# USharma002/CUDA-PathTracer

Hardware: AMD Instinct MI355X
Metric: Msamples/s (higher is better)
Workload: dtype f32; 1 GPU; c2: cbox.obj 1024x1024, 256 spp, max_depth 8, default camera, seed 2023 (BASELINE configs[1]); width=1024, height=1024, spp=256, max_depth=8, segments_per_launch=default, parallelism=tile1, frames=one ptmi_render_frame call per step

## Files before the change

cuda-pathtracer_amd/csrc/bounce.h:

```cpp
#pragma once
#include "shading.h"
#include "sweep_records.h"

namespace ptmi {

struct BounceArgs {
    DeviceScene sc; TileMap tm; PathState st; FrameParams fp;
    const int* queue_in; int n_in;
    const int* count_in;
    int* queue_out; int* count_out;
    int segments;
    StatCounters* stats;
    int many_waves;
    int* done_count;
    int* next_count;
    int* host_count;
    int* cursor;
    unsigned int* cost; unsigned int* cost_max;
};

using BounceKernel = void (*)(BounceArgs);
#pragma GCC visibility push(hidden)
BounceKernel select_bounce_sync(const BounceArgs& a);
BounceKernel select_bounce_phased(const BounceArgs& a);
BounceKernel select_bounce_wide(const BounceArgs& a);
#pragma GCC visibility pop

inline bool is_guided(const BounceArgs& a) { return a.fp.sampling_mode != 0 && a.sc.cdfs != nullptr; }

#ifdef PTMI_TRACE_WAVES
#define PTMI_TR(...) __VA_ARGS__
#else
#define PTMI_TR(...)
#endif

template <bool LDS_GEOM, bool SWEEP_RECORDS = false>
__device__ __forceinline__ float4* stage_scene(const DeviceScene& sc, float4* lds, const float4*& nodes, const float4*& prims, const float4*& mats) {
    static_assert(LDS_GEOM || !SWEEP_RECORDS, "the sweep's records exist in LDS only");
    nodes = sc.nodes; prims = sc.prims; mats = sc.mats;
    if (LDS_GEOM) {
        const int n_node_vec = 2 * sc.n_nodes, n_prim_vec = sc.prim_stride * sc.n_prims, n_mat_vec = 3 * sc.n_prims;
        if (SWEEP_RECORDS) {
            ptmi_sweep_prepare(reinterpret_cast<const ptmi_vec_bits*>(sc.nodes), sc.n_nodes, reinterpret_cast<const ptmi_vec_bits*>(sc.prims),
                               sc.prim_stride, sc.n_prims, reinterpret_cast<ptmi_vec_bits*>(lds), reinterpret_cast<ptmi_vec_bits*>(lds + n_node_vec),
                               lds_address(lds), (int)threadIdx.x, kBlock);
        } else {
            for (int i = threadIdx.x; i < n_node_vec; i += kBlock) lds[i] = sc.nodes[i];
            for (int i = threadIdx.x; i < n_prim_vec; i += kBlock) lds[n_node_vec + i] = sc.prims[i];
        }
        for (int i = threadIdx.x; i < n_mat_vec; i += kBlock) lds[n_node_vec + n_prim_vec + i] = sc.mats[i];
        nodes = lds; prims = lds + n_node_vec; mats = lds + n_node_vec + n_prim_vec;
        lds += n_node_vec + n_prim_vec + n_mat_vec;
        __syncthreads();
    }
    return lds;
}

template <bool STATS, bool COMPACT = true>
__device__ __forceinline__ void finish_launch(const BounceArgs& a, bool alive, int slot, const LaneCounters& cn) {
    if (COMPACT) {
        const unsigned long long mask = __ballot(alive);
        const int lane = threadIdx.x & 63;
        int base = 0;
        if (lane == 0 && mask) base = atomicAdd(a.count_out, __popcll(mask));
        base = __shfl(base, 0);
        if (alive) a.queue_out[base + __popcll(mask & ((1ull << lane) - 1ull))] = slot;
    }
    if (STATS) {
        unsigned long long r = cn.rays, nv = cn.node_visits, pt = cn.prim_tests, h = cn.hits, tv = cn.top_visits;
        unsigned long long cc = cn.cert_chain, cf = cn.cert_fallback;
        for (int off = 32; off > 0; off >>= 1) {
            r += __shfl_down(r, off); nv += __shfl_down(nv, off); pt += __shfl_down(pt, off); h += __shfl_down(h, off); tv += __shfl_down(tv, off);
            cc += __shfl_down(cc, off); cf += __shfl_down(cf, off);
        }
        if ((threadIdx.x & 63) == 0) {
            atomicAdd(&a.stats->rays, r); atomicAdd(&a.stats->node_visits, nv);
            atomicAdd(&a.stats->prim_tests, pt); atomicAdd(&a.stats->hits, h);
            if (tv) atomicAdd(&a.stats->top_node_visits, tv);
            if (cc) atomicAdd(&a.stats->cert_chain, cc);
            if (cf) atomicAdd(&a.stats->cert_fallback, cf);
        }
    }
}

__device__ __forceinline__ void publish_count(const BounceArgs& a) {
    if (!a.host_count) return;
    if ((threadIdx.x & 63) == 0) {
        __threadfence();
        if (atomicAdd(a.done_count, 1) == (int)(gridDim.x * (kBlock / 64)) - 1) {
            const int c = atomicAdd(a.count_out, 0);
            atomicExch(a.next_count, 0); atomicExch(a.next_count + 1, 0);
            atomicExch(a.done_count, 0);
            __hip_atomic_store(a.host_count, c, __ATOMIC_RELEASE, __HIP_MEMORY_SCOPE_SYSTEM);
        }
    }
}

__device__ __forceinline__ bool end_visit(const BounceArgs& a, int n_in, bool more, int& slot, PathRegs& p, int& segs_left) {
    store_path(a.st, slot, p);
    if (a.cost) {
        const unsigned int c = a.cost[slot] + (unsigned int)(a.segments - segs_left);
        a.cost[slot] = c;
        if (!more) atomicMax(a.cost_max, c);
    }
    const int lane = threadIdx.x & 63;
    const unsigned long long ending = __ballot(1), surviving = __ballot(more);
    const int first = __ffsll((long long)ending) - 1;
    int out_base = 0, in_base = 0;
    if (lane == first) {
        if (surviving) out_base = atomicAdd(a.count_out, __popcll(surviving));
        if (a.cursor) in_base = atomicAdd(a.cursor, __popcll(ending));
    }
    out_base = __shfl(out_base, first); in_base = __shfl(in_base, first);
    if (more) a.queue_out[out_base + __popcll(surviving & ((1ull << lane) - 1ull))] = slot;
    const int entry = (int)(gridDim.x * kBlock) + in_base + __popcll(ending & ((1ull << lane) - 1ull));
    if (!(a.cursor && entry < n_in)) return false;
    slot = a.queue_in ? a.queue_in[entry] : entry;
    load_path(a.st, a.tm, slot, p);
    segs_left = a.segments;
    return true;
}

}
```

cuda-pathtracer_amd/csrc/bounce_sync.hip:

```cpp
#include "bounce.h"

namespace ptmi {

template <int MODE, bool LDS_GEOM, bool HAS_QUADS, bool STATS, bool GUIDED, bool BATCH>
__device__ __forceinline__ void bounce_body(const BounceArgs& a) {
    extern __shared__ float4 smem[];
    static_assert(MODE != TRAVERSAL_SWEEP || LDS_GEOM, "the sweep reads the scene through LDS broadcasts");
    const int n_in = a.count_in ? *a.count_in : a.n_in;
    if ((int)(blockIdx.x * kBlock) >= n_in) return;
    const int idx = blockIdx.x * kBlock + threadIdx.x;
    const bool active = idx < n_in;
    const float4 *nodes, *prims, *mats;
    float4* lds = stage_scene<LDS_GEOM, MODE == TRAVERSAL_SWEEP>(a.sc, smem, nodes, prims, mats);
    int* stack = reinterpret_cast<int*>(lds) + threadIdx.x;
    if (GUIDED) fill_grid_solid_angles();

    const int slot = active ? (a.queue_in ? a.queue_in[idx] : idx) : 0;
    bool alive = active;
    PathRegs p = {};
    if (active) load_path(a.st, a.tm, slot, p);
    LaneCounters cn = {0, 0, 0, 0, 0, 0, 0};

    for (int seg = 0; seg < a.segments; seg++) {
        if (!__any(alive)) break;
        float t = 0.0f; int k = -1;
        if (STATS && alive) cn.rays++;
        const bool hit = scene_intersect<MODE, HAS_QUADS, STATS>(nodes, prims, a.sc.prim_stride, a.sc.n_nodes, stack, alive,
                                                               p.o, p.d, 1e-4f, FLT_MAX, t, k, cn);
        constexpr bool LEAN = MODE == TRAVERSAL_SWEEP && !STATS && !GUIDED;
        if (alive) alive = shade_step<STATS, GUIDED, false, BATCH, LEAN>(a.fp, a.tm, MatSource{mats, nullptr, nullptr}, a.sc.cdfs, p, hit, t, k, cn, slot);
    }

    if (active) store_path(a.st, slot, p);
    finish_launch<STATS>(a, alive, slot, cn);
}
template <int MODE, bool LDS_GEOM, bool HAS_QUADS, bool STATS, bool GUIDED, bool BATCH>
__global__ __launch_bounds__(kBlock, GUIDED ? 6 : ((BATCH || (HAS_QUADS && !STATS)) && MODE == TRAVERSAL_SWEEP ? 8 : 1)) __attribute__((amdgpu_num_sgpr(80))) void ptmi_bounce(BounceArgs a) {
    bounce_body<MODE, LDS_GEOM, HAS_QUADS, STATS, GUIDED, BATCH>(a);
    publish_count(a);
}

BounceKernel select_bounce_sync(const BounceArgs& a) {
    const auto pick = [&](auto mode, auto geom) {
        return with_bool(a.sc.has_quads, [&](auto quads) {
            return with_bool(a.stats != nullptr, [&](auto stats) {
                return with_bool(is_guided(a), [&](auto guided) {
                    return with_bool(a.fp.n_frames > 1, [&](auto batch) -> BounceKernel {
                        return ptmi_bounce<decltype(mode)::value, decltype(geom)::value, decltype(quads)::value, decltype(stats)::value,
                                           decltype(guided)::value, decltype(batch)::value>;
                    });
                });
            });
        });
    };
    switch (a.sc.traversal) {
        case TRAVERSAL_SWEEP: return pick(std::integral_constant<int, TRAVERSAL_SWEEP>{}, std::true_type{});
        case TRAVERSAL_LANE: return with_bool(a.sc.lds_resident, [&](auto geom) { return pick(std::integral_constant<int, TRAVERSAL_LANE>{}, geom); });
        default: return with_bool(a.sc.lds_resident, [&](auto geom) { return pick(std::integral_constant<int, TRAVERSAL_STACK>{}, geom); });
    }
}

}
```

cuda-pathtracer_amd/csrc/kernels.hip:

```cpp
#include "bounce.h"

namespace ptmi {

__global__ __launch_bounds__(kBlock) void ptmi_render_init(TileMap tm, PathState st, const uint32_t* __restrict__ jump,
                                                           unsigned long long seed_base) {
    __shared__ uint32_t M[160 * 5];
    const int n = tm.local_rows * tm.width;
    const int slot = blockIdx.x * kBlock + threadIdx.x;
    const bool live = slot < n;
    int x = 0, y = 0;
    const unsigned int pix = live ? (unsigned int)global_pixel(tm, slot, x, y) : 0u;
    const unsigned long long seed = seed_base + (unsigned long long)pix;
    const uint32_t s0 = ((uint32_t)seed) ^ 0xaad26b49u;
    const uint32_t s1 = (uint32_t)(seed >> 32) ^ 0xf7dcefddu;
    const uint32_t t0 = 1099087573u * s0;
    const uint32_t t1 = 2591861531u * s1;
    uint32_t v[5] = {123456789u + t0, 362436069u ^ t0, 521288629u + t1, 88675123u ^ t1, 5783321u + t0};
    const uint32_t d = 6615241u + t1 + t0;

    for (int k = 0; k < 32; k++) {
        const bool mine = live && ((pix >> k) & 1u);
        if (!__syncthreads_or(mine ? 1 : 0)) continue;
        for (int i = threadIdx.x; i < 160 * 5; i += kBlock) M[i] = jump[k * 160 * 5 + i];
        __syncthreads();
        if (mine) {
            uint32_t r[5] = {0u, 0u, 0u, 0u, 0u};
#pragma unroll
            for (int w = 0; w < 5; w++) {
                const uint32_t word = v[w];
                for (int b = 0; b < 32; b++) {
                    const uint32_t m = 0u - ((word >> b) & 1u);
                    const uint32_t* row = &M[(w * 32 + b) * 5];
                    r[0] ^= row[0] & m; r[1] ^= row[1] & m; r[2] ^= row[2] & m; r[3] ^= row[3] & m; r[4] ^= row[4] & m;
                }
            }
#pragma unroll
            for (int w = 0; w < 5; w++) v[w] = r[w];
        }
        __syncthreads();
    }
    if (!live) return;
    st.E[slot] = make_uint4(v[0], v[1], v[2], v[3]);
    st.F[slot] = make_uint2(v[4], d);
    st.A[slot] = make_float4(0, 0, 0, 1.0f);
    st.B[slot] = make_float4(0, 0, 1.0f, 1.0f);
    st.C[slot] = make_float4(0, 0, 0, 1.0f);
    st.D[slot] = make_float4(0, 0, 0, __uint_as_float(0u));
}

__global__ __launch_bounds__(kBlock) void ptmi_frame_begin(TileMap tm, PathState st, FrameParams fp) {
    const int n = tm.local_rows * tm.width;
    const int slot = blockIdx.x * kBlock + threadIdx.x;
    if (slot >= n) return;
    int x, y;
    global_pixel(tm, slot, x, y);
    const uint4 e = st.E[slot]; const uint2 f = st.F[slot];
    Rng rng = {e.x, e.y, e.z, e.w, f.x, f.y};
    f3 o, d;
    camera_ray(fp, tm, x, y, rng, o, d);
    st.A[slot] = make_float4(o.x, o.y, o.z, 1.0f);
    st.B[slot] = make_float4(d.x, d.y, d.z, 1.0f);
    st.C[slot] = make_float4(0.0f, 0.0f, 0.0f, 1.0f);
    st.D[slot] = make_float4(0.0f, 0.0f, 0.0f, __uint_as_float(0u));
    st.E[slot] = make_uint4(rng.v0, rng.v1, rng.v2, rng.v3);
    st.F[slot] = make_uint2(rng.v4, rng.d);
}

size_t bounce_lds_bytes_wide(const DeviceScene& sc) { return (size_t)sc.w_top * kWideNodeDwords * 4 + (size_t)sc.w_depth * kBlock * sizeof(uint2); }
size_t bounce_lds_bytes(const DeviceScene& sc) {
    if (sc.traversal == TRAVERSAL_WIDE || sc.traversal == TRAVERSAL_CERTIFIED) return bounce_lds_bytes_wide(sc);
    size_t b = 0;
    const bool geom = sc.lds_resident || sc.traversal == TRAVERSAL_SWEEP;
    if (geom) b += ptmi_scene_lds_vecs(sc.n_nodes, sc.prim_stride, sc.n_prims) * sizeof(float4);
    if (sc.traversal == TRAVERSAL_STACK) b += (size_t)sc.stack_entries * kBlock * sizeof(int);
    return b;
}

static BounceKernel select_bounce_kernel(const BounceArgs& a, size_t* lds) {
    const DeviceScene& sc = a.sc;
    *lds = bounce_lds_bytes(sc);
    switch (sc.traversal) {
        case TRAVERSAL_PHASED: return select_bounce_phased(a);
        case TRAVERSAL_PACKED: *lds = (size_t)sc.n_top * 2 * sizeof(float4); return select_bounce_phased(a);
        case TRAVERSAL_WIDE:
        case TRAVERSAL_CERTIFIED: return select_bounce_wide(a);
        default: return select_bounce_sync(a);
    }
}

void launch_bounce(const DeviceScene& sc, const TileMap& tm, const PathState& st, const FrameParams& fp,
                   const int* queue_in, int n_in, const int* count_in, int* queue_out, int* count_out, int segments,
                   StatCounters* stats, bool many_waves, hipStream_t s, const CountPublish& pub, const LaunchSchedule& sched) {
    if (n_in <= 0) return;
    BounceArgs a{sc, tm, st, fp, queue_in, n_in, count_in, queue_out, count_out, segments, stats, many_waves ? 1 : 0,
                 pub.done_count, pub.next_count, pub.host_count, nullptr, nullptr, nullptr};
    dim3 grid((n_in + kBlock - 1) / kBlock);
    const bool wide = sc.traversal == TRAVERSAL_WIDE || sc.traversal == TRAVERSAL_CERTIFIED;
    if (wide && sched.max_waves > 0 && sched.cursor) {
        a.cursor = sched.cursor;
        grid.x = std::min<unsigned int>(grid.x, (unsigned int)(sched.max_waves + kBlock / 64 - 1) / (kBlock / 64));
    }
    if (wide) { a.cost = sched.cost; a.cost_max = sched.cost_max; }
    size_t lds = 0;
    const BounceKernel k = select_bounce_kernel(a, &lds);
    hipLaunchKernelGGL(k, grid, dim3(kBlock), lds, s, a);
}

int bounce_resident_waves(const DeviceScene& sc, const FrameParams& fp, bool stats, int n_cus) {
    BounceArgs a{sc, TileMap(), PathState(), fp, nullptr, 0, nullptr, nullptr, nullptr, 0, stats ? reinterpret_cast<StatCounters*>(1) : nullptr, 0,
                 nullptr, nullptr, nullptr, nullptr, nullptr, nullptr};
    size_t lds = 0;
    const BounceKernel k = select_bounce_kernel(a, &lds);
    int blocks = 0;
    if (hipOccupancyMaxActiveBlocksPerMultiprocessor(&blocks, k, kBlock, lds) != hipSuccess) blocks = 0;
    return blocks * (kBlock / 64) * n_cus;
}

__device__ __forceinline__ int cost_class(unsigned int c, unsigned int cmax, int shift) {
    const unsigned long long k = ((unsigned long long)min(c, cmax) << 8) / ((unsigned long long)cmax + 1ull);
    return (255 - (int)k) >> shift;
}
__global__ __launch_bounds__(kBlock) void ptmi_cost_histogram(const int* __restrict__ queue_in, int n, const unsigned int* __restrict__ cost,
                                                              const unsigned int* __restrict__ cost_max, int* __restrict__ hist, int shift) {
    __shared__ int h[256];
    h[threadIdx.x] = 0;
    __syncthreads();
    const unsigned int cmax = *cost_max;
    for (int i = blockIdx.x * kBlock + threadIdx.x; i < n; i += gridDim.x * kBlock)
        atomicAdd(&h[cost_class(cost[queue_in ? queue_in[i] : i], cmax, shift)], 1);
    __syncthreads();
    if (h[threadIdx.x]) atomicAdd(&hist[threadIdx.x], h[threadIdx.x]);
}
__global__ __launch_bounds__(kBlock) void ptmi_cost_offsets(int* __restrict__ hist) {
    __shared__ int h[256];
    h[threadIdx.x] = hist[threadIdx.x];
    __syncthreads();
    if (threadIdx.x == 0) { int acc = 0; for (int c = 0; c < 256; c++) { const int v = h[c]; h[c] = acc; acc += v; } }
    __syncthreads();
    hist[256 + threadIdx.x] = h[threadIdx.x];
}
__global__ __launch_bounds__(kBlock) void ptmi_cost_scatter(const int* __restrict__ queue_in, int n, const unsigned int* __restrict__ cost,
                                                            const unsigned int* __restrict__ cost_max, int* __restrict__ hist, int* __restrict__ queue, int shift) {
    __shared__ int h[256], base[256];
    __shared__ unsigned char cls[kBlock];
    h[threadIdx.x] = 0;
    const int i = blockIdx.x * kBlock + threadIdx.x;
    const int entry = i < n ? (queue_in ? queue_in[i] : i) : 0;
    const int c = i < n ? cost_class(cost[entry], *cost_max, shift) : 255;
    cls[threadIdx.x] = (unsigned char)c;
    __syncthreads();
    if (i < n) atomicAdd(&h[c], 1);
    int local = 0;
    for (int j = 0; j < (int)threadIdx.x; j++) local += cls[j] == c ? 1 : 0;
    __syncthreads();
    if (h[threadIdx.x]) base[threadIdx.x] = atomicAdd(&hist[256 + threadIdx.x], h[threadIdx.x]);
    __syncthreads();
    if (i < n) queue[base[c] + local] = entry;
}
void launch_order_by_cost(const int* queue_in, int n, const unsigned int* cost, const unsigned int* cost_max, int* hist, int* queue, int classes, hipStream_t s) {
    if (n <= 0) return;
    int shift = 0;
    while ((256 >> shift) > classes && shift < 7) shift++;
    (void)hipMemsetAsync(hist, 0, 512 * sizeof(int), s);
    const int blocks = (n + kBlock - 1) / kBlock;
    hipLaunchKernelGGL(ptmi_cost_histogram, dim3(std::min(blocks, 1024)), dim3(kBlock), 0, s, queue_in, n, cost, cost_max, hist, shift);
    hipLaunchKernelGGL(ptmi_cost_offsets, dim3(1), dim3(kBlock), 0, s, hist);
    hipLaunchKernelGGL(ptmi_cost_scatter, dim3(blocks), dim3(kBlock), 0, s, queue_in, n, cost, cost_max, hist, queue, shift);
}

void launch_render_init(const TileMap& tm, const PathState& st, const uint32_t* d_jump, uint64_t seed_base, hipStream_t s) {
    const int n = tm.local_rows * tm.width;
    if (n <= 0) return;
    hipLaunchKernelGGL(ptmi_render_init, dim3((n + kBlock - 1) / kBlock), dim3(kBlock), 0, s, tm, st, d_jump,
                       (unsigned long long)seed_base);
}

void launch_frame_begin(const TileMap& tm, const PathState& st, const FrameParams& fp, hipStream_t s) {
    const int n = tm.local_rows * tm.width;
    if (n <= 0) return;
    hipLaunchKernelGGL(ptmi_frame_begin, dim3((n + kBlock - 1) / kBlock), dim3(kBlock), 0, s, tm, st, fp);
}

__global__ __launch_bounds__(kBlock) void ptmi_resolve(TileMap tm, PathState st, int spp, unsigned char* __restrict__ rgb8,
                                                       float* __restrict__ radiance, const float4* __restrict__ color_src) {
    const int n = tm.local_rows * tm.width;
    const int slot = blockIdx.x * kBlock + threadIdx.x;
    if (slot >= n) return;
    const float4 D = color_src ? color_src[slot] : st.D[slot];
    int ox, olr;
    slot_to_local(tm, slot, ox, olr);
    const size_t out = (size_t)olr * (size_t)tm.width + (size_t)ox;
    const float k = rcp_rn((float)spp);
    resolve_pixel(D, k, out, rgb8, radiance);
}

void launch_resolve(const TileMap& tm, const PathState& st, int spp, unsigned char* rgb8, float* radiance, hipStream_t s,
                    const float4* color_src) {
    const int n = tm.local_rows * tm.width;
    if (n <= 0) return;
    hipLaunchKernelGGL(ptmi_resolve, dim3((n + kBlock - 1) / kBlock), dim3(kBlock), 0, s, tm, st, spp, rgb8, radiance, color_src);
}

__global__ __launch_bounds__(kBlock) void ptmi_pass_begin(TileMap tm, PathState st, FrameParams fp, const int* __restrict__ queue, int n, int first) {
    const int idx = blockIdx.x * kBlock + threadIdx.x;
    if (idx >= n) return;
    const int slot = queue ? queue[idx] : idx;
    int x, y;
    global_pixel(tm, slot, x, y);
    const uint4 e = st.E[slot]; const uint2 f = st.F[slot];
    Rng rng = {e.x, e.y, e.z, e.w, f.x, f.y};
    f3 o, d;
    camera_ray(fp, tm, x, y, rng, o, d);
    const float4 D = first ? make_float4(0.0f, 0.0f, 0.0f, 0.0f) : st.D[slot];
    st.A[slot] = make_float4(o.x, o.y, o.z, 1.0f);
    st.B[slot] = make_float4(d.x, d.y, d.z, 1.0f);
    st.C[slot] = make_float4(0.0f, 0.0f, 0.0f, 1.0f);
    st.D[slot] = make_float4(D.x, D.y, D.z, __uint_as_float(0u));
    st.E[slot] = make_uint4(rng.v0, rng.v1, rng.v2, rng.v3);
    st.F[slot] = make_uint2(rng.v4, rng.d);
}

__global__ __launch_bounds__(kBlock) void ptmi_adapt(PathState st, AccumBuffers ab, AdaptRule rule, const int* __restrict__ queue_in, int n,
                                                     int* __restrict__ queue_out, int* __restrict__ count_out) {
    const int idx = blockIdx.x * kBlock + threadIdx.x;
    const bool active = idx < n;
    const int slot = active ? (queue_in ? queue_in[idx] : idx) : 0;
    bool more = false;
    if (active) {
        const float4 S = st.D[slot];
        const float4 prev = rule.first ? make_float4(0.0f, 0.0f, 0.0f, 0.0f) : ab.prev[slot];
        float M2 = rule.first ? 0.0f : ab.m2[slot];
        const unsigned int k = (rule.first ? 0u : ab.passes[slot]) + 1u;
        const float dx = S.x - prev.x, dy = S.y - prev.y, dz = S.z - prev.z;
        const float y = (0.2126f * dx + 0.7152f * dy + 0.0722f * dz) * rule.inv_spp;
        const float nf = (float)k;
        const float delta = y - prev.w;
        const float mean = prev.w + delta / nf;
        M2 = M2 + delta * (y - mean);
        const float a = rule.threshold * (mean + rule.floor_);
        const bool stop = rule.stopping && ((int)k >= rule.max_passes ||
                                            ((int)k >= rule.min_passes && M2 <= a * a * (float)(k * (k - 1u))));
        ab.prev[slot] = make_float4(S.x, S.y, S.z, mean);
        ab.m2[slot] = M2;
        ab.passes[slot] = k;
        more = !stop;
    }
    const unsigned long long mask = __ballot(more);
    const int lane = threadIdx.x & 63;
    int base = 0;
    if (lane == 0 && mask) base = atomicAdd(count_out, __popcll(mask));
    base = __shfl(base, 0);
    if (more) queue_out[base + __popcll(mask & ((1ull << lane) - 1ull))] = slot;
}

__global__ __launch_bounds__(kBlock) void ptmi_resolve_counts(TileMap tm, PathState st, const unsigned int* __restrict__ passes, int spp,
                                                              unsigned char* __restrict__ rgb8, float* __restrict__ radiance,
                                                              unsigned int* __restrict__ counts) {
    const int n = tm.local_rows * tm.width;
    const int slot = blockIdx.x * kBlock + threadIdx.x;
    if (slot >= n) return;
    const float4 D = st.D[slot];
    int ox, olr;
    slot_to_local(tm, slot, ox, olr);
    const size_t out = (size_t)olr * (size_t)tm.width + (size_t)ox;
    const unsigned int samples = passes[slot] * (unsigned int)spp;
    counts[out] = samples;
    resolve_pixel(D, rcp_rn((float)samples), out, rgb8, radiance);
}

void launch_pass_begin(const TileMap& tm, const PathState& st, const FrameParams& fp, const int* queue, int n, bool first, hipStream_t s) {
    if (n <= 0) return;
    hipLaunchKernelGGL(ptmi_pass_begin, dim3((n + kBlock - 1) / kBlock), dim3(kBlock), 0, s, tm, st, fp, queue, n, first ? 1 : 0);
}
void launch_adapt(const PathState& st, const AccumBuffers& ab, const AdaptRule& rule, const int* queue_in, int n, int* queue_out,
                  int* count_out, hipStream_t s) {
    if (n <= 0) return;
    hipLaunchKernelGGL(ptmi_adapt, dim3((n + kBlock - 1) / kBlock), dim3(kBlock), 0, s, st, ab, rule, queue_in, n, queue_out, count_out);
}
void launch_resolve_counts(const TileMap& tm, const PathState& st, const unsigned int* passes, int spp, unsigned char* rgb8,
                           float* radiance, unsigned int* counts, hipStream_t s) {
    const int n = tm.local_rows * tm.width;
    if (n <= 0) return;
    hipLaunchKernelGGL(ptmi_resolve_counts, dim3((n + kBlock - 1) / kBlock), dim3(kBlock), 0, s, tm, st, passes, spp, rgb8, radiance, counts);
}

}
```

cuda-pathtracer_amd/csrc/pt_device.h:

```cpp
#pragma once
#include "device_scene.h"
#include "wide_bvh.h"

#include <float.h>

#include <type_traits>

#include "../../include/ptmi_math.h"

namespace ptmi {

template <typename F>
static decltype(auto) with_bool(bool b, F&& f) {
    return b ? f(std::true_type{}) : f(std::false_type{});
}

struct Rng { uint32_t v0, v1, v2, v3, v4, d; };

__device__ __forceinline__ uint32_t rng_next(Rng& r) {
    const uint32_t t = r.v0 ^ (r.v0 >> 2);
    r.v0 = r.v1; r.v1 = r.v2; r.v2 = r.v3; r.v3 = r.v4;
    r.v4 = (r.v4 ^ (r.v4 << 4)) ^ (t ^ (t << 1));
    r.d += 362437u;
    return r.v4 + r.d;
}
__device__ __forceinline__ float rng_uniform(Rng& r) {
    const uint32_t x = rng_next(r);
    return (float)x * 2.3283064e-10f + (2.3283064e-10f / 2.0f);
}

__device__ __forceinline__ float min_raw(float a, float b) { float r; asm("v_min_f32 %0, %1, %2" : "=v"(r) : "v"(a), "v"(b)); return r; }
__device__ __forceinline__ float max_raw(float a, float b) { float r; asm("v_max_f32 %0, %1, %2" : "=v"(r) : "v"(a), "v"(b)); return r; }
__device__ __forceinline__ float min3_raw(float a, float b, float c) { float r; asm("v_min3_f32 %0, %1, %2, %3" : "=v"(r) : "v"(a), "v"(b), "v"(c)); return r; }
__device__ __forceinline__ float max3_raw(float a, float b, float c) { float r; asm("v_max3_f32 %0, %1, %2, %3" : "=v"(r) : "v"(a), "v"(b), "v"(c)); return r; }

__device__ __forceinline__ float mt_candidate(f3 v0, f3 edge1, f3 edge2, f3 o, f3 d, float eps_for_a, float t_lo) {
    const f3 h = cross(d, edge2);
    const float a = dot(edge1, h);
    const float f = rcp_exact_normal(a);
    const f3 s = o - v0;
    const float u = f * dot(s, h);
    const float m1 = min3_raw(fabsf(a) - eps_for_a, u, 1.0f - u);
    if (!__any(m1 >= 0.0f)) return __builtin_inff();
    const f3 q = cross(s, edge1);
    const float v = f * dot(d, q);
    const float t = f * dot(edge2, q);
    float m = min3_raw(m1, v, 1.0f - (u + v));
    m = min_raw(m, t - t_lo);
    return (m >= 0.0f) ? t : __builtin_inff();
}
__device__ __forceinline__ bool mt_accept(f3 v0, f3 edge1, f3 edge2, f3 o, f3 d, float eps_for_a, float t_lo, float closest_t, float& t) {
    const f3 h = cross(d, edge2);
    const float a = dot(edge1, h);
    const float f = rcp_exact_normal(a);
    const f3 s = o - v0;
    const float u = f * dot(s, h);
    const float m1 = min3_raw(fabsf(a) - eps_for_a, u, 1.0f - u);
    if (!__any(m1 >= 0.0f)) return false;
    const f3 q = cross(s, edge1);
    const float v = f * dot(d, q);
    t = f * dot(edge2, q);
    float m = min3_raw(m1, v, 1.0f - (u + v));
    m = min_raw(m, t - t_lo);
    return (m >= 0.0f) & (t < closest_t);
}
__device__ __forceinline__ bool mt_hit(f3 v0, f3 edge1, f3 edge2, f3 o, f3 d, float eps_for_a, float t_lo, float& t) {
    const f3 h = cross(d, edge2);
    const float a = dot(edge1, h);
    const float f = rcp_exact_normal(a);
    const f3 s = o - v0;
    const float u = f * dot(s, h);
    const float m1 = min3_raw(fabsf(a) - eps_for_a, u, 1.0f - u);
    if (!__any(m1 >= 0.0f)) return false;
    const f3 q = cross(s, edge1);
    const float v = f * dot(d, q);
    t = f * dot(edge2, q);
    float m = min3_raw(m1, v, 1.0f - (u + v));
    m = min_raw(m, t - t_lo);
    return m >= 0.0f;
}
__device__ __forceinline__ float mt_t_lo(float t_min) {
    const float eps_up = __uint_as_float(__float_as_uint(1e-8f) + 1u);
    return t_min > 1e-8f ? t_min : eps_up;
}

__device__ __forceinline__ f3 xyz(const float4& v) { return mk3(v.x, v.y, v.z); }
struct f3p { float x, y, z; };

__device__ __forceinline__ void build_frame(f3 n, f3& t, f3& b) {
    if (n.z < -0.9999999f) { t = mk3(0.0f, -1.0f, 0.0f); b = mk3(-1.0f, 0.0f, 0.0f); return; }
    const float a = rcp_rn(1.0f + n.z);
    const float c = -n.x * n.y * a;
    t = mk3(1.0f - n.x * n.x * a, c, -n.x);
    b = mk3(c, 1.0f - n.y * n.y * a, -n.y);
}

__device__ __forceinline__ float dot_from_zero(f3 a, f3 b) { float s = 0.0f; s += a.x * b.x; s += a.y * b.y; s += a.z * b.z; return s; }

__device__ __forceinline__ int direction_to_grid_index_local(f3 world_dir, f3 normal) {
    f3 tangent, bitangent;
    build_frame(normal, tangent, bitangent);
    const float lx = dot_from_zero(world_dir, tangent), ly = dot_from_zero(world_dir, bitangent), lz = dot(world_dir, normal);
    const float r = sqrt_rn(lx * lx + ly * ly + lz * lz);
    const float theta = (r > 0.0f) ? ptmi_acosf(fminf(lz / r, 1.0f)) : 0.0f;
    float phi = ptmi_atan2f(ly, lx);
    if (phi < 0.0f) phi = (float)((double)phi + (double)2.0f * PTMI_PI_D);
    int grid_theta = (int)fminf((float)(((double)theta / PTMI_PI_D) * kGridRes), (float)(kGridRes - 1));
    int grid_phi = (int)fminf((float)(((double)phi / ((double)2.0f * PTMI_PI_D)) * kGridRes), (float)(kGridRes - 1));
    grid_theta = max(0, min(grid_theta, kGridRes - 1));
    grid_phi = max(0, min(grid_phi, kGridRes - 1));
    return grid_theta * kGridRes + grid_phi;
}

__device__ __forceinline__ void resolve_pixel(const float4& D, float k, size_t out, unsigned char* __restrict__ rgb8,
                                              float* __restrict__ radiance) {
    const float c[3] = {D.x * k, D.y * k, D.z * k};
    const float gamma = 1.0f / 2.2f;
#pragma unroll
    for (int ch = 0; ch < 3; ch++) {
        if (radiance) radiance[out * 3 + ch] = c[ch];
        if (rgb8) {
            const float tm_ = c[ch] / (c[ch] + 1.0f);
            const float g = ptmi_powf(tm_, gamma);
            rgb8[out * 3 + ch] = (unsigned char)(255.99f * fminf(g, 1.0f));
        }
    }
}

}
```

cuda-pathtracer_amd/csrc/shading.h:

```cpp
#pragma once
#include "pt_device.h"
#include "shade_lean.h"
#include "traversal.h"

namespace ptmi {

__device__ __forceinline__ void slot_to_local(const TileMap& tm, int slot, int& x, int& lr) {
    if (tm.tile8) {
        const int tile = slot >> 6, in = slot & 63;
        const int tiles_per_row = tm.width >> 3;
        const int ty = tile / tiles_per_row, tx = tile - ty * tiles_per_row;
        lr = (ty << 3) + (in >> 3);
        x = (tx << 3) + (in & 7);
    } else {
        lr = slot / tm.width;
        x = slot - lr * tm.width;
    }
}
__device__ __forceinline__ int global_pixel(const TileMap& tm, int slot, int& x, int& y) {
    int lr;
    slot_to_local(tm, slot, x, lr);
    y = ((lr / tm.row_block) * tm.n_ranks + tm.rank) * tm.row_block + (lr % tm.row_block);
    return y * tm.width + x;
}

__device__ __forceinline__ f3 camera_dir_raw(const FrameParams& fp, float u, float v, f3& o) {
    const f3 org = mk3(fp.cam_origin[0], fp.cam_origin[1], fp.cam_origin[2]);
    const f3 llc = mk3(fp.cam_llc[0], fp.cam_llc[1], fp.cam_llc[2]);
    const f3 hor = mk3(fp.cam_hor[0], fp.cam_hor[1], fp.cam_hor[2]);
    const f3 ver = mk3(fp.cam_ver[0], fp.cam_ver[1], fp.cam_ver[2]);
    o = org;
    return llc + u * hor + v * ver - org;
}
__device__ __forceinline__ float div_by_size(float a, float W, float inv) {
    if (inv != 0.0f) return ptmi_div_by_size_lean(a, W, inv);
    return a / W;
}
template <bool LEAN = false>
__device__ __forceinline__ f3 camera_dir_raw(const FrameParams& fp, const TileMap& tm, int x, int y, float r1, float r2, f3& o) {
    const float u = LEAN ? div_by_size((float)x + r1, (float)tm.width, tm.inv_width) : ((float)x + r1) / (float)tm.width;
    const float v = LEAN ? div_by_size((float)y + r2, (float)tm.height, tm.inv_height) : ((float)y + r2) / (float)tm.height;
    return camera_dir_raw(fp, u, v, o);
}
__device__ __forceinline__ void camera_ray_uv(const FrameParams& fp, float u, float v, f3& o, f3& d) {
    d = unit_vector(camera_dir_raw(fp, u, v, o));
}
__device__ __forceinline__ void camera_ray(const FrameParams& fp, const TileMap& tm, int x, int y, Rng& rng, f3& o, f3& d) {
    const float r1 = rng_uniform(rng);
    const float r2 = rng_uniform(rng);
    d = unit_vector(camera_dir_raw(fp, tm, x, y, r1, r2, o));
}

__device__ __forceinline__ void sincos_2pi_lean(float phi, float* s, float* c) {
    const bool outside = __float_as_uint(phi) > PTMI_TWO_PI_F_BITS;
    const bool flagged = ptmi_sincos_2pi_fast(phi, s, c) != 0;
    if (__any(outside || flagged)) ptmi_sincosf(phi, s, c);
}

template <bool LEAN = false>
__device__ __forceinline__ f3 cosine_hemisphere(f3 n, float u, float v) {
    const float r = sqrt_lean(u);
    const float phi = (float)((double)2.0f * PTMI_PI_D * (double)v);
    float sphi, cphi;
    if (LEAN) sincos_2pi_lean(phi, &sphi, &cphi);
    else ptmi_sincosf(phi, &sphi, &cphi);
    const float x = r * cphi;
    const float y = r * sphi;
    const float z = sqrt_lean(fmaxf(0.0f, 1.0f - u));
    f3 tangent, bitangent;
    if (n.z < -0.9999999f) {
        tangent = mk3(0.0f, -1.0f, 0.0f);
        bitangent = mk3(-1.0f, 0.0f, 0.0f);
    } else {
        const float a = rcp_exact_normal(1.0f + n.z);
        const float b = -n.x * n.y * a;
        tangent = mk3(1.0f - n.x * n.x * a, b, -n.x);
        bitangent = mk3(b, 1.0f - n.y * n.y * a, -n.y);
    }
    return unit_vector_lean(x * tangent + y * bitangent + z * n);
}

struct PathRegs {
    f3 o, d, tp, L, color;
    Rng rng;
    unsigned int sample_idx;
    int depth, px, py;
};

__device__ __forceinline__ void load_path(const PathState& st, const TileMap& tm, int slot, PathRegs& p) {
    const float4 A = st.A[slot], B = st.B[slot], C = st.C[slot], D = st.D[slot];
    const uint4 E = st.E[slot]; const uint2 F = st.F[slot];
    p.o = xyz(A); p.d = xyz(B); p.L = xyz(C); p.color = xyz(D);
    p.tp = mk3(A.w, B.w, C.w);
    const unsigned int meta = __float_as_uint(D.w);
    p.sample_idx = meta >> 8; p.depth = (int)(meta & 0xffu);
    p.rng = Rng{E.x, E.y, E.z, E.w, F.x, F.y};
    global_pixel(tm, slot, p.px, p.py);
}
__device__ __forceinline__ void store_path(const PathState& st, int slot, const PathRegs& p) {
    st.A[slot] = make_float4(p.o.x, p.o.y, p.o.z, p.tp.x);
    st.B[slot] = make_float4(p.d.x, p.d.y, p.d.z, p.tp.y);
    st.C[slot] = make_float4(p.L.x, p.L.y, p.L.z, p.tp.z);
    st.D[slot] = make_float4(p.color.x, p.color.y, p.color.z, __uint_as_float((p.sample_idx << 8) | (unsigned int)p.depth));
    st.E[slot] = make_uint4(p.rng.v0, p.rng.v1, p.rng.v2, p.rng.v3);
    st.F[slot] = make_uint2(p.rng.v4, p.rng.d);
}

__device__ __forceinline__ int linear_search_cdf(const float* __restrict__ cdf, int size, float xi) {
    xi = fminf(fmaxf(xi, 0.0f), 0.999999f);
    int r = size - 1;
    for (int i = size - 1; i >= 0; i--) if (xi < cdf[i]) r = i;
    return r;
}
__shared__ float g_grid_solid_angle[8];
__device__ __forceinline__ void fill_grid_solid_angles() {
    if (threadIdx.x < 8) {
        const int theta_idx = threadIdx.x;
        const float theta_center = (float)((double)(((float)theta_idx + 0.5f) * 0.125f) * (PTMI_PI_D * 0.5f));
        float st, ct;
        ptmi_sincosf(theta_center, &st, &ct);
        const float sin_theta = fmaxf(st, 0.01f);
        const float solid_angle = (float)(((double)sin_theta * ((PTMI_PI_D * 0.5f) / 8)) * (2.0f * PTMI_PI_D / 16));
        g_grid_solid_angle[theta_idx] = fmaxf(solid_angle, 1e-6f);
    }
    __syncthreads();
}
__device__ __forceinline__ float grid_pdf_for_cell(const float* __restrict__ g, int theta_idx, int phi_idx) {
    const float cell_value = g[kCdfPdf + theta_idx * 16 + phi_idx];
    if (cell_value < 1e-8f) return 1e-6f;
    const float cell_prob = cell_value / fmaxf(g[kCdfTotal], 1e-6f);
    return cell_prob / g_grid_solid_angle[theta_idx];
}
__device__ __forceinline__ f3 grid_sample(const float* __restrict__ g, f3 normal, Rng& rng, float& out_pdf) {
    const float xi1 = rng_uniform(rng);
    const float xi2 = rng_uniform(rng);
    const int theta_idx = linear_search_cdf(g + kCdfMarginal, 8, xi1);
    const int phi_idx = linear_search_cdf(g + kCdfRowCdfs + theta_idx * 16, 16, xi2);
    const float jitter_theta = rng_uniform(rng);
    const float jitter_phi = rng_uniform(rng);
    float theta = (float)((double)(((float)theta_idx + jitter_theta) * 0.125f) * (PTMI_PI_D * 0.5f));
    theta = fminf(theta, (float)(PTMI_PI_D * 0.5f - (double)0.01f));
    const float phi = (float)((double)((((float)phi_idx + jitter_phi) * 0.0625f) * 2.0f) * PTMI_PI_D);
    float sin_t, cos_t, sin_p, cos_p;
    ptmi_sincosf(theta, &sin_t, &cos_t);
    ptmi_sincosf(phi, &sin_p, &cos_p);
    f3 tangent, bitangent;
    build_frame(normal, tangent, bitangent);
    const f3 world = unit_vector((sin_t * cos_p) * tangent + (sin_t * sin_p) * bitangent + cos_t * normal);
    out_pdf = grid_pdf_for_cell(g, theta_idx, phi_idx);
    return world;
}
__device__ __forceinline__ float grid_compute_pdf(const float* __restrict__ g, f3 dir, f3 normal) {
    f3 tangent, bitangent;
    build_frame(normal, tangent, bitangent);
    const float lx = dot_from_zero(dir, tangent), ly = dot_from_zero(dir, bitangent), lz = dot(dir, normal);
    const float theta = ptmi_acosf(fminf(fmaxf(lz, -1.0f), 1.0f));
    float phi = ptmi_atan2f(ly, lx);
    if (phi < 0.0f) phi = (float)((double)phi + (double)2.0f * PTMI_PI_D);
    if ((double)theta > PTMI_PI_D * 0.5f) return 0.0f;
    int theta_idx = (int)(((double)theta * ((double)2.0f / PTMI_PI_D)) * 8);
    int phi_idx = (int)(((double)phi * ((double)0.5f / PTMI_PI_D)) * 16);
    theta_idx = max(0, min(theta_idx, 7));
    phi_idx = max(0, min(phi_idx, 15));
    return grid_pdf_for_cell(g, theta_idx, phi_idx);
}
__device__ __forceinline__ float mis_power_heuristic(float pdf_a, float pdf_b) {
    if (pdf_a <= 0.0f) return 0.0f;
    const float a2 = pdf_a * pdf_a, b2 = pdf_b * pdf_b;
    return a2 / (a2 + b2);
}
__device__ __forceinline__ f3 sample_mis(const float* __restrict__ g, f3 normal, Rng& rng, float& weight, float bsdf_prob) {
    const float BSDF_PROB = fmaxf(fminf(bsdf_prob, 0.99f), 0.01f);
    const float GRID_PROB = 1.0f - BSDF_PROB;
    const float xi = rng_uniform(rng);
    f3 dir;
    if (xi < BSDF_PROB) {
        const float u = rng_uniform(rng), v = rng_uniform(rng);
        dir = cosine_hemisphere(normal, u, v);
        const float cos_theta = fmaxf(dot(dir, normal), 0.0f);
        const float pdf_bsdf = (float)((double)cos_theta / PTMI_PI_D);
        const float pdf_grid = grid_compute_pdf(g, dir, normal);
        const float mis_w = mis_power_heuristic(pdf_bsdf, pdf_grid);
        weight = (pdf_bsdf > 1e-6f) ? mis_w / BSDF_PROB : 0.0f;
    } else {
        float pdf_grid;
        dir = grid_sample(g, normal, rng, pdf_grid);
        const float cos_theta = fmaxf(dot(dir, normal), 0.0f);
        const float pdf_bsdf = (float)((double)cos_theta / PTMI_PI_D);
        const float mis_w = mis_power_heuristic(pdf_grid, pdf_bsdf);
        if (pdf_grid > 1e-6f && cos_theta > 0.0f) {
            const float w = (float)((double)(mis_w * cos_theta) / ((PTMI_PI_D * (double)pdf_grid) * (double)GRID_PROB));
            weight = fminf(w, 10.0f);
        } else weight = 0.0f;
    }
    return dir;
}

struct MatSource { const float4* mats; const float4* mtab; const int* load_index; int stride = 1; };
template <bool PACKED>
__device__ __forceinline__ void fetch_material(const MatSource& ms, int k, f3& n, f3& bsdf, f3& Le, int& row) {
    if (PACKED) {
        const float4 m = ms.mats[(size_t)k * ms.stride];
        n = xyz(m); row = __float_as_int(m.w);
        bsdf = xyz(ms.mtab[2 * row]); Le = xyz(ms.mtab[2 * row + 1]);
    } else {
        const float4 m = ms.mats[3 * k];
        n = xyz(m); row = __float_as_int(m.w);
        bsdf = xyz(ms.mats[3 * k + 1]); Le = xyz(ms.mats[3 * k + 2]);
    }
}
template <bool STATS, bool GUIDED, bool PACKED = false, bool BATCH = false, bool LEAN = false>
__device__ __forceinline__ bool shade_step(const FrameParams& fp, const TileMap& tm, const MatSource& ms, const float* cdfs, PathRegs& p,
                                           bool hit, float t, int k, LaneCounters& cn, int slot) {
    bool end_sample = !hit;
    bool go_on = false;
    f3 hp, sn;
    if (hit) {
        if (STATS) cn.hits++;
        f3 n, bsdf, Le; int row;
        fetch_material<PACKED>(ms, k, n, bsdf, Le, row);
        hp = p.o + t * p.d;
        p.L = p.L + p.tp * Le;
        if (p.depth > 2) {
            const float max_tp = fmaxf(p.tp.x, fmaxf(p.tp.y, p.tp.z));
            const float rr_prob = fminf(max_tp, 0.95f);
            if (rng_uniform(p.rng) > rr_prob) end_sample = true;
            else {
                const float inv_rr = LEAN ? rcp_exact_normal(rr_prob) : rcp_rn(rr_prob);
                p.tp = mk3(p.tp.x * inv_rr, p.tp.y * inv_rr, p.tp.z * inv_rr);
            }
        }
        if (!end_sample) {
            p.tp = p.tp * bsdf;
            if (length_below_1em5(length_squared(p.tp))) end_sample = true;
            else {
                sn = dot(p.d, n) < 0 ? n : -n;
                const float* g = nullptr;
                if (GUIDED) {
                    const float* rec = cdfs + (size_t)(PACKED ? ms.load_index[k] : row) * kCdfDwords;
                    if (__float_as_int(rec[kCdfValid]) != 0) g = rec;
                }
                if (GUIDED && g) {
                    f3 next;
                    float weight = 1.0f;
                    if (fp.sampling_mode == 3) {
                        next = sample_mis(g, sn, p.rng, weight, fp.mis_bsdf_fraction);
                    } else {
                        float grid_pdf;
                        next = grid_sample(g, sn, p.rng, grid_pdf);
                        const float cos_theta = fmaxf(dot(next, sn), 0.0f);
                        weight = (float)((double)cos_theta / (PTMI_PI_D * (double)fmaxf(grid_pdf, 1e-6f)));
                        weight = fminf(fmaxf(weight, 0.0f), 10.0f);
                    }
                    p.tp = mk3(p.tp.x * weight, p.tp.y * weight, p.tp.z * weight);
                    p.depth++;
                    if (p.depth < fp.max_depth) {
                        p.o = hp + 1e-4f * sn;
                        p.d = unit_vector(next);
                    } else end_sample = true;
                } else if (GUIDED) {
                    const float u = rng_uniform(p.rng);
                    const float v = rng_uniform(p.rng);
                    p.depth++;
                    if (p.depth < fp.max_depth) {
                        const f3 next = cosine_hemisphere(sn, u, v);
                        p.o = hp + 1e-4f * sn;
                        p.d = unit_vector(next);
                    } else end_sample = true;
                } else {
                    p.depth++;
                    if (p.depth < fp.max_depth) go_on = true;
                    else {
                        rng_next(p.rng); rng_next(p.rng);
                        end_sample = true;
                    }
                }
            }
        }
    }
    if (end_sample) {
        p.color = p.color + p.L;
        p.sample_idx++;
        if (!BATCH) {
            if (p.sample_idx >= (unsigned int)fp.spp) return false;
        } else if ((p.sample_idx & fp.sample_mask) >= (unsigned int)fp.spp) {
            const unsigned int frame = p.sample_idx >> 16;
            if (frame + 1u >= (unsigned int)fp.n_frames) return false;
            fp.frame_color[frame * (unsigned int)fp.n_local + (unsigned int)slot] = make_float4(p.color.x, p.color.y, p.color.z, 0.0f);
            p.sample_idx = (frame + 1u) << 16;
            p.color = mk3(0.0f, 0.0f, 0.0f);
        }
        if (GUIDED) {
            camera_ray(fp, tm, p.px, p.py, p.rng, p.o, p.d);
            p.tp = mk3(1.0f, 1.0f, 1.0f); p.L = mk3(0.0f, 0.0f, 0.0f); p.depth = 0;
        }
    }
    if (!GUIDED) {
        const float r1 = rng_uniform(p.rng);
        const float r2 = rng_uniform(p.rng);
        f3 w;
        if (go_on) {
            w = cosine_hemisphere<LEAN>(sn, r1, r2);
            p.o = hp + 1e-4f * sn;
        } else {
            w = camera_dir_raw<LEAN>(fp, tm, p.px, p.py, r1, r2, p.o);
            p.tp = mk3(1.0f, 1.0f, 1.0f); p.L = mk3(0.0f, 0.0f, 0.0f); p.depth = 0;
        }
        p.d = LEAN ? unit_vector_voted(w) : unit_vector(w);
    }
    return true;
}

}
```

cuda-pathtracer_amd/python/ptmi_buildinfo.py:

```python
import hashlib
import os

_HERE = os.path.dirname(os.path.abspath(__file__))
PKG = os.path.dirname(_HERE)
ROOT = os.path.dirname(PKG)

def _csrc(*names):
    return [os.path.join(PKG, "csrc", n) for n in names]


_SHARED_SOURCES = _csrc("pt_device.h", "pt_vec.h", "device_scene.h", "wide_bvh.h", "wide_walk.h", "prim_sample.h") + [
    os.path.join(ROOT, "include", "ptmi_math.h"), os.path.join(PKG, "Makefile")]
KERNEL_SOURCES = _csrc("kernels.hip", "bounce_sync.hip", "bounce_phased.hip", "bounce_wide.hip", "first_hit.hip", "debug_hooks.hip",
                       "traversal.h", "sweep_records.h", "shading.h", "shade_lean.h", "bounce.h") + _SHARED_SOURCES + [
    os.path.join(PKG, "host", "render_run.cpp"), os.path.join(PKG, "host", "launch_rule.h"),
    os.path.join(PKG, "host", "wide_bvh.cpp"),
]
SOLVER_SOURCES = _csrc("radiosity.hip", "form_factors.hip", "anyhit.h") + _SHARED_SOURCES + [os.path.join(PKG, "host", "radiosity_state.cpp")]


def _sha(paths):
    h = hashlib.sha256()
    for p in paths:
        h.update(os.path.basename(p).encode() + b"\0")
        with open(p, "rb") as f:
            h.update(f.read())
    return h.hexdigest()


def lib_sha256():
    p = os.environ.get("PTMI_LIB") or os.path.join(PKG, "libptmi.so")
    if not os.path.exists(p):
        return None
    with open(p, "rb") as f:
        return hashlib.sha256(f.read()).hexdigest()


def kernel_src_sha256():
    return _sha(KERNEL_SOURCES)


def solver_src_sha256():
    return _sha(SOLVER_SOURCES)


def stamps():
    return {"lib_sha256": lib_sha256(), "kernel_src_sha256": kernel_src_sha256(), "solver_src_sha256": solver_src_sha256()}


def profile_is_current(profile, solver=False):
    if profile.get("lib_sha256") and profile.get("lib_sha256") == lib_sha256():
        return True, "lib"
    if solver:
        if profile.get("solver_src_sha256") and profile.get("solver_src_sha256") == solver_src_sha256():
            return True, "solver_sources"
        return False, None
    if profile.get("kernel_src_sha256") and profile.get("kernel_src_sha256") == kernel_src_sha256():
        return True, "kernel_sources"
    return False, None
```

Before: 8080 Msamples/s.

## Add lean sweep shading step with LDS camera block and branchless RNG

Adds a specialised shade_step_sweep for the lean sweep traversal path. The new step makes the Russian-roulette draw branchless (rng_uniform_if), pulls two RNG values in one fused step, and always draws the next direction's random pair whether the path continues or restarts. Camera parameters and image sizes are packed into a 4-vector frame block in LDS next to the materials, so camera-ray generation reads LDS broadcasts and uses a scalar wave-uniform flag for the division path. The aim is to cut divergent branches and scalar-parameter loads per bounce, at the cost of a little more LDS and a possible change in the RNG stream order.

```diff
diff --git a/cuda-pathtracer_amd/csrc/bounce.h b/cuda-pathtracer_amd/csrc/bounce.h
--- a/cuda-pathtracer_amd/csrc/bounce.h
+++ b/cuda-pathtracer_amd/csrc/bounce.h
@@ -1,6 +1,7 @@
 #pragma once
 #include "shading.h"
 #include "sweep_records.h"
+#include "frame_block.h"
 
 namespace ptmi {
 
@@ -35,26 +36,33 @@
 #endif
 
 template <bool LDS_GEOM, bool SWEEP_RECORDS = false>
-__device__ __forceinline__ float4* stage_scene(const DeviceScene& sc, float4* lds, const float4*& nodes, const float4*& prims, const float4*& mats) {
+__device__ __forceinline__ float4* stage_scene(const DeviceScene& sc, float4* lds, const float4*& nodes, const float4*& prims, const float4*& mats,
+                                               const FrameParams* fp = nullptr, const TileMap* tm = nullptr) {
     static_assert(LDS_GEOM || !SWEEP_RECORDS, "the sweep's records exist in LDS only");
     nodes = sc.nodes; prims = sc.prims; mats = sc.mats;
     if (LDS_GEOM) {
         const int n_node_vec = 2 * sc.n_nodes, n_prim_vec = sc.prim_stride * sc.n_prims, n_mat_vec = 3 * sc.n_prims;
+        const int mats_at = n_node_vec + n_prim_vec + (SWEEP_RECORDS ? PTMI_FRAME_BLOCK_VECS : 0);
         if (SWEEP_RECORDS) {
             ptmi_sweep_prepare(reinterpret_cast<const ptmi_vec_bits*>(sc.nodes), sc.n_nodes, reinterpret_cast<const ptmi_vec_bits*>(sc.prims),
                                sc.prim_stride, sc.n_prims, reinterpret_cast<ptmi_vec_bits*>(lds), reinterpret_cast<ptmi_vec_bits*>(lds + n_node_vec),
                                lds_address(lds), (int)threadIdx.x, kBlock);
+            if (fp && threadIdx.x == kBlock - 1)
+                ptmi_frame_block_pack(fp->cam_origin, fp->cam_llc, fp->cam_hor, fp->cam_ver, tm->width, tm->height, tm->inv_width, tm->inv_height,
+                                      reinterpret_cast<ptmi_vec_bits*>(lds + n_node_vec + n_prim_vec));
         } else {
             for (int i = threadIdx.x; i < n_node_vec; i += kBlock) lds[i] = sc.nodes[i];
             for (int i = threadIdx.x; i < n_prim_vec; i += kBlock) lds[n_node_vec + i] = sc.prims[i];
         }
-        for (int i = threadIdx.x; i < n_mat_vec; i += kBlock) lds[n_node_vec + n_prim_vec + i] = sc.mats[i];
-        nodes = lds; prims = lds + n_node_vec; mats = lds + n_node_vec + n_prim_vec;
-        lds += n_node_vec + n_prim_vec + n_mat_vec;
+        for (int i = threadIdx.x; i < n_mat_vec; i += kBlock) lds[mats_at + i] = sc.mats[i];
+        nodes = lds; prims = lds + n_node_vec; mats = lds + mats_at;
+        lds += mats_at + n_mat_vec;
         __syncthreads();
     }
     return lds;
 }
+
+__device__ __forceinline__ const float4* frame_block_of(const float4* mats) { return mats - PTMI_FRAME_BLOCK_VECS; }
 
 template <bool STATS, bool COMPACT = true>
 __device__ __forceinline__ void finish_launch(const BounceArgs& a, bool alive, int slot, const LaneCounters& cn) {
diff --git a/cuda-pathtracer_amd/csrc/bounce_sync.hip b/cuda-pathtracer_amd/csrc/bounce_sync.hip
--- a/cuda-pathtracer_amd/csrc/bounce_sync.hip
+++ b/cuda-pathtracer_amd/csrc/bounce_sync.hip
@@ -1,4 +1,11 @@
 #include "bounce.h"
+
+#ifndef PTMI_SWEEP_FRAME_BLOCK
+#define PTMI_SWEEP_FRAME_BLOCK 1
+#endif
+#ifndef PTMI_SWEEP_LATE
+#define PTMI_SWEEP_LATE 1
+#endif
 
 namespace ptmi {
 
@@ -11,7 +18,14 @@
     const int idx = blockIdx.x * kBlock + threadIdx.x;
     const bool active = idx < n_in;
     const float4 *nodes, *prims, *mats;
-    float4* lds = stage_scene<LDS_GEOM, MODE == TRAVERSAL_SWEEP>(a.sc, smem, nodes, prims, mats);
+    float4* lds;
+    if constexpr (MODE == TRAVERSAL_SWEEP) lds = stage_scene<LDS_GEOM, true>(a.sc, smem, nodes, prims, mats, &a.fp, &a.tm);
+    else lds = stage_scene<LDS_GEOM>(a.sc, smem, nodes, prims, mats);
+    constexpr bool LEAN = MODE == TRAVERSAL_SWEEP && !STATS && !GUIDED;
+    constexpr bool LATE = LEAN && PTMI_SWEEP_LATE;
+    constexpr bool FRAME = LATE && PTMI_SWEEP_FRAME_BLOCK;
+    FrameBlock fb;
+    if constexpr (FRAME) fb = frame_block(frame_block_of(mats), a.tm);
     int* stack = reinterpret_cast<int*>(lds) + threadIdx.x;
     if (GUIDED) fill_grid_solid_angles();
 
@@ -27,8 +41,11 @@
         if (STATS && alive) cn.rays++;
         const bool hit = scene_intersect<MODE, HAS_QUADS, STATS>(nodes, prims, a.sc.prim_stride, a.sc.n_nodes, stack, alive,
                                                                p.o, p.d, 1e-4f, FLT_MAX, t, k, cn);
-        constexpr bool LEAN = MODE == TRAVERSAL_SWEEP && !STATS && !GUIDED;
-        if (alive) alive = shade_step<STATS, GUIDED, false, BATCH, LEAN>(a.fp, a.tm, MatSource{mats, nullptr, nullptr}, a.sc.cdfs, p, hit, t, k, cn, slot);
+        if constexpr (LATE) {
+            if (alive) alive = shade_step_sweep<BATCH, FRAME>(a.fp, a.tm, fb, mats, p, hit, t, k, slot);
+        } else {
+            if (alive) alive = shade_step<STATS, GUIDED, false, BATCH, LEAN>(a.fp, a.tm, MatSource{mats, nullptr, nullptr}, a.sc.cdfs, p, hit, t, k, cn, slot);
+        }
     }
 
     if (active) store_path(a.st, slot, p);
diff --git a/cuda-pathtracer_amd/csrc/frame_block.h b/cuda-pathtracer_amd/csrc/frame_block.h
--- /dev/null
+++ b/cuda-pathtracer_amd/csrc/frame_block.h
@@ -0,0 +1,23 @@
+#ifndef PTMI_FRAME_BLOCK_H
+#define PTMI_FRAME_BLOCK_H
+
+#include "sweep_records.h"
+
+#define PTMI_FRAME_BLOCK_VECS 4
+
+PTMI_HD size_t ptmi_sweep_lds_vecs(int n_nodes, int prim_stride, int n_prims) {
+    return ptmi_scene_lds_vecs(n_nodes, prim_stride, n_prims) + PTMI_FRAME_BLOCK_VECS;
+}
+
+PTMI_HD uint32_t ptmi_f2u(float x) { uint32_t u; __builtin_memcpy(&u, &x, 4); return u; }
+
+PTMI_HD void ptmi_frame_block_pack(const float org[3], const float llc[3], const float hor[3], const float ver[3], int width, int height,
+                                   float inv_width, float inv_height, ptmi_vec_bits out[PTMI_FRAME_BLOCK_VECS]) {
+    const ptmi_vec_bits v0 = {ptmi_f2u(llc[0]), ptmi_f2u(llc[1]), ptmi_f2u(llc[2]), ptmi_f2u((float)width)};
+    const ptmi_vec_bits v1 = {ptmi_f2u(hor[0]), ptmi_f2u(hor[1]), ptmi_f2u(hor[2]), ptmi_f2u(inv_width)};
+    const ptmi_vec_bits v2 = {ptmi_f2u(ver[0]), ptmi_f2u(ver[1]), ptmi_f2u(ver[2]), ptmi_f2u((float)height)};
+    const ptmi_vec_bits v3 = {ptmi_f2u(org[0]), ptmi_f2u(org[1]), ptmi_f2u(org[2]), ptmi_f2u(inv_height)};
+    out[0] = v0; out[1] = v1; out[2] = v2; out[3] = v3;
+}
+
+#endif
diff --git a/cuda-pathtracer_amd/csrc/kernels.hip b/cuda-pathtracer_amd/csrc/kernels.hip
--- a/cuda-pathtracer_amd/csrc/kernels.hip
+++ b/cuda-pathtracer_amd/csrc/kernels.hip
@@ -71,7 +71,8 @@
     if (sc.traversal == TRAVERSAL_WIDE || sc.traversal == TRAVERSAL_CERTIFIED) return bounce_lds_bytes_wide(sc);
     size_t b = 0;
     const bool geom = sc.lds_resident || sc.traversal == TRAVERSAL_SWEEP;
-    if (geom) b += ptmi_scene_lds_vecs(sc.n_nodes, sc.prim_stride, sc.n_prims) * sizeof(float4);
+    if (geom) b += (sc.traversal == TRAVERSAL_SWEEP ? ptmi_sweep_lds_vecs(sc.n_nodes, sc.prim_stride, sc.n_prims)
+                                                    : ptmi_scene_lds_vecs(sc.n_nodes, sc.prim_stride, sc.n_prims)) * sizeof(float4);
     if (sc.traversal == TRAVERSAL_STACK) b += (size_t)sc.stack_entries * kBlock * sizeof(int);
     return b;
 }
diff --git a/cuda-pathtracer_amd/csrc/pt_device.h b/cuda-pathtracer_amd/csrc/pt_device.h
--- a/cuda-pathtracer_amd/csrc/pt_device.h
+++ b/cuda-pathtracer_amd/csrc/pt_device.h
@@ -27,6 +27,29 @@
 __device__ __forceinline__ float rng_uniform(Rng& r) {
     const uint32_t x = rng_next(r);
     return (float)x * 2.3283064e-10f + (2.3283064e-10f / 2.0f);
+}
+
+__device__ __forceinline__ float rng_uniform_if(Rng& r, bool draw) {
+    const uint32_t t = r.v0 ^ (r.v0 >> 2);
+    const uint32_t v = (r.v4 ^ (r.v4 << 4)) ^ (t ^ (t << 1));
+    const uint32_t d = r.d + 362437u;
+    r.v0 = draw ? r.v1 : r.v0; r.v1 = draw ? r.v2 : r.v1; r.v2 = draw ? r.v3 : r.v2; r.v3 = draw ? r.v4 : r.v3;
+    r.v4 = draw ? v : r.v4; r.d = draw ? d : r.d;
+    return (float)(v + d) * 2.3283064e-10f + (2.3283064e-10f / 2.0f);
+}
+__device__ __forceinline__ void rng_next2(Rng& r, uint32_t& x1, uint32_t& x2) {
+    const uint32_t t1 = r.v0 ^ (r.v0 >> 2), t2 = r.v1 ^ (r.v1 >> 2);
+    const uint32_t a = (r.v4 ^ (r.v4 << 4)) ^ (t1 ^ (t1 << 1));
+    const uint32_t b = (a ^ (a << 4)) ^ (t2 ^ (t2 << 1));
+    r.v0 = r.v2; r.v1 = r.v3; r.v2 = r.v4; r.v3 = a; r.v4 = b;
+    r.d += 362437u; x1 = a + r.d;
+    r.d += 362437u; x2 = b + r.d;
+}
+__device__ __forceinline__ void rng_uniform2(Rng& r, float& u1, float& u2) {
+    uint32_t x1, x2;
+    rng_next2(r, x1, x2);
+    u1 = (float)x1 * 2.3283064e-10f + (2.3283064e-10f / 2.0f);
+    u2 = (float)x2 * 2.3283064e-10f + (2.3283064e-10f / 2.0f);
 }
 
 __device__ __forceinline__ float min_raw(float a, float b) { float r; asm("v_min_f32 %0, %1, %2" : "=v"(r) : "v"(a), "v"(b)); return r; }
diff --git a/cuda-pathtracer_amd/csrc/shading.h b/cuda-pathtracer_amd/csrc/shading.h
--- a/cuda-pathtracer_amd/csrc/shading.h
+++ b/cuda-pathtracer_amd/csrc/shading.h
@@ -32,15 +32,36 @@
     o = org;
     return llc + u * hor + v * ver - org;
 }
-__device__ __forceinline__ float div_by_size(float a, float W, float inv) {
-    if (inv != 0.0f) return ptmi_div_by_size_lean(a, W, inv);
+__device__ __forceinline__ float div_by_size(float a, float W, float inv, bool lean) {
+    if (lean) return ptmi_div_by_size_lean(a, W, inv);
     return a / W;
 }
+__device__ __forceinline__ float div_by_size(float a, float W, float inv) { return div_by_size(a, W, inv, inv != 0.0f); }
 template <bool LEAN = false>
 __device__ __forceinline__ f3 camera_dir_raw(const FrameParams& fp, const TileMap& tm, int x, int y, float r1, float r2, f3& o) {
     const float u = LEAN ? div_by_size((float)x + r1, (float)tm.width, tm.inv_width) : ((float)x + r1) / (float)tm.width;
     const float v = LEAN ? div_by_size((float)y + r2, (float)tm.height, tm.inv_height) : ((float)y + r2) / (float)tm.height;
     return camera_dir_raw(fp, u, v, o);
+}
+struct FrameBlock {
+    const float4* v = nullptr;
+    int lean_sizes = 0;
+};
+__device__ __forceinline__ FrameBlock frame_block(const float4* v, const TileMap& tm) {
+    int lean_sizes = ((__float_as_uint(tm.inv_width) << 1) != 0u ? 1 : 0) | ((__float_as_uint(tm.inv_height) << 1) != 0u ? 2 : 0);
+    lean_sizes = __builtin_amdgcn_readfirstlane(lean_sizes);
+    asm("" : "+s"(lean_sizes));
+    return FrameBlock{v, lean_sizes};
+}
+__device__ __forceinline__ f3 camera_dir_block(const FrameBlock& fb, int x, int y, float r1, float r2, f3& o) {
+    const float4 b0 = fb.v[0], b1 = fb.v[1], b2 = fb.v[2], b3 = fb.v[3];
+    const float a = (float)x + r1, b = (float)y + r2;
+    int lean_sizes = fb.lean_sizes;
+    asm volatile("" : "+s"(lean_sizes));
+    const float u = div_by_size(a, b0.w, b1.w, (lean_sizes & 1) != 0);
+    const float v = div_by_size(b, b2.w, b3.w, (lean_sizes & 2) != 0);
+    o = xyz(b3);
+    return xyz(b0) + u * xyz(b1) + v * xyz(b2) - xyz(b3);
 }
 __device__ __forceinline__ void camera_ray_uv(const FrameParams& fp, float u, float v, f3& o, f3& d) {
     d = unit_vector(camera_dir_raw(fp, u, v, o));
@@ -311,4 +332,55 @@
     return true;
 }
 
-}
+template <bool BATCH, bool FRAME>
+__device__ __forceinline__ bool shade_step_sweep(const FrameParams& fp, const TileMap& tm, const FrameBlock& fb, const float4* mats, PathRegs& p,
+                                                 bool hit, float t, int k, int slot) {
+    f3 n, bsdf, Le; int row;
+    fetch_material<false>(MatSource{mats, nullptr, nullptr}, hit ? k : 0, n, bsdf, Le, row);
+    const f3 hp = p.o + t * p.d;
+    if (hit) p.L = p.L + p.tp * Le;
+    asm("" : "+v"(p.L.x), "+v"(p.L.y), "+v"(p.L.z), "+v"(p.tp.x), "+v"(p.tp.y), "+v"(p.tp.z));
+    const bool deep = hit && p.depth > 2;
+    const float rr_prob = fminf(fmaxf(p.tp.x, fmaxf(p.tp.y, p.tp.z)), 0.95f);
+    const bool killed = deep && rng_uniform_if(p.rng, deep) > rr_prob;
+    const float inv_rr = rcp_exact_normal(rr_prob);
+    if (deep && !killed) p.tp = mk3(p.tp.x * inv_rr, p.tp.y * inv_rr, p.tp.z * inv_rr);
+    bool end_sample = !hit || killed;
+    if (!end_sample) p.tp = p.tp * bsdf;
+    end_sample = end_sample || length_below_1em5(length_squared(p.tp));
+    const f3 sn = dot(p.d, n) < 0 ? n : -n;
+    if (!end_sample) p.depth++;
+    const bool go_on = !end_sample && p.depth < fp.max_depth;
+    if (!end_sample && !go_on) {
+        uint32_t x1, x2;
+        rng_next2(p.rng, x1, x2);
+    }
+    if (!go_on) {
+        p.color = p.color + p.L;
+        p.sample_idx++;
+        p.tp = mk3(1.0f, 1.0f, 1.0f); p.L = mk3(0.0f, 0.0f, 0.0f); p.depth = 0;
+        if (!BATCH) {
+            if (p.sample_idx >= (unsigned int)fp.spp) return false;
+        } else if ((p.sample_idx & fp.sample_mask) >= (unsigned int)fp.spp) {
+            const unsigned int frame = p.sample_idx >> 16;
+            if (frame + 1u >= (unsigned int)fp.n_frames) return false;
+            fp.frame_color[frame * (unsigned int)fp.n_local + (unsigned int)slot] = make_float4(p.color.x, p.color.y, p.color.z, 0.0f);
+            p.sample_idx = (frame + 1u) << 16;
+            p.color = mk3(0.0f, 0.0f, 0.0f);
+        }
+    }
+    float r1, r2;
+    rng_uniform2(p.rng, r1, r2);
+    f3 w;
+    if (go_on) {
+        w = cosine_hemisphere<true>(sn, r1, r2);
+        p.o = hp + 1e-4f * sn;
+    } else {
+        w = FRAME ? camera_dir_block(fb, p.px, p.py, r1, r2, p.o)
+                  : camera_dir_raw<true>(fp, tm, p.px, p.py, r1, r2, p.o);
+    }
+    p.d = unit_vector_voted(w);
+    return true;
+}
+
+}
diff --git a/cuda-pathtracer_amd/python/ptmi_buildinfo.py b/cuda-pathtracer_amd/python/ptmi_buildinfo.py
--- a/cuda-pathtracer_amd/python/ptmi_buildinfo.py
+++ b/cuda-pathtracer_amd/python/ptmi_buildinfo.py
@@ -12,7 +12,7 @@
 _SHARED_SOURCES = _csrc("pt_device.h", "pt_vec.h", "device_scene.h", "wide_bvh.h", "wide_walk.h", "prim_sample.h") + [
     os.path.join(ROOT, "include", "ptmi_math.h"), os.path.join(PKG, "Makefile")]
 KERNEL_SOURCES = _csrc("kernels.hip", "bounce_sync.hip", "bounce_phased.hip", "bounce_wide.hip", "first_hit.hip", "debug_hooks.hip",
-                       "traversal.h", "sweep_records.h", "shading.h", "shade_lean.h", "bounce.h") + _SHARED_SOURCES + [
+                       "traversal.h", "sweep_records.h", "frame_block.h", "shading.h", "shade_lean.h", "bounce.h") + _SHARED_SOURCES + [
     os.path.join(PKG, "host", "render_run.cpp"), os.path.join(PKG, "host", "launch_rule.h"),
     os.path.join(PKG, "host", "wide_bvh.cpp"),
 ]
```

Result: faster. 8247 Msamples/s (median of 6 runs) (+2.1%).
